# CHAINNEVERLIU/Pytorch-RL-EnhancedStableBaselines

Hardware: AMD Instinct MI355X
Metric: env-steps/sec (SAC, two-series CSTR, 4096 vec-envs) at 1/2/4/8 GPUs (higher is better)
Workload: dtype f32; 1 GPU; SAC MlpPolicy class defaults on 4096 vectorised two-series CSTR envs per GPU (obs 4/act 2, euler, batch 256, ring 244x4096, 1 gradient step per vec-step; hipGraph replay, 8 iterations per graph); n_envs_per_gpu=4096, global_batch=256, parallelism=dp1, hip_graph=True, hip_graph_requested=True, graph_unroll=8, blas=rocblas, n_updates=2370

## Files before the change

### pytorch-rl-enhancedstablebaselines_amd/csrc/cstr_chain.hip

```cpp
#include <hip/hip_runtime.h>
#include <stdint.h>

#include "../../include/cstr_rl_hip.h"
#include "cstr_device.h"
#include "cstr_rng_device.h"

namespace {

using f32x4 = __attribute__((ext_vector_type(4))) float;
typedef unsigned int u32x4 __attribute__((ext_vector_type(4)));
constexpr int BUF_OOB = 0x40000000;
constexpr int CH_THREADS = 256, CH_WAVES = 4;
constexpr float LOG_STD_MIN = -20.0f, LOG_STD_MAX = 2.0f;
constexpr int MAX_A = CSTR_MAX_HEAD_ACT;

constexpr int SM_PART = 0;
constexpr int SM_RED = SM_PART + 3 * 64 * 4;
constexpr int SM_XS = SM_RED + 4 * 16 * 8;
constexpr int SM_GS = SM_XS + 16 * 16;
constexpr int SM_PANEL = SM_GS + 16 * 8;
static size_t chain_lds_bytes(int k, int w1_pad) { return (size_t)(SM_PANEL + 16 * (k + 4) + w1_pad * k) * sizeof(float); }

__device__ __forceinline__ __amdgpu_buffer_rsrc_t rsrc_of(const float *base, const int64_t floats)
{
    return __builtin_amdgcn_make_buffer_rsrc(const_cast<float *>(base), 0, (int)(floats * 4), 0x00020000);
}

__device__ __forceinline__ float4 ld128(const __amdgpu_buffer_rsrc_t rs, const int byte_off)
{
    const u32x4 v = __builtin_amdgcn_raw_buffer_load_b128(rs, byte_off, 0, 0);
    return make_float4(__uint_as_float(v.x), __uint_as_float(v.y), __uint_as_float(v.z), __uint_as_float(v.w));
}

__device__ __forceinline__ float ld32(const __amdgpu_buffer_rsrc_t rs, const int byte_off)
{
    return __uint_as_float(__builtin_amdgcn_raw_buffer_load_b32(rs, byte_off, 0, 0));
}

template <int WX> __device__ __forceinline__ constexpr int exact_h1() { return WX == 1 ? 256 : 400; }
template <int WX> __device__ __forceinline__ constexpr int exact_h2() { return WX == 1 ? 256 : 300; }
template <int NQ, int WX> __device__ __forceinline__ constexpr int exact_tiles() { return WX == 1 ? NQ / 4 : (NQ >= 8 ? NQ / 8 : 1); }

#ifdef CSTR_CHAIN_STAMPS
__device__ unsigned long long chain_stamps[4 * 1024 * 4 * 8];
#define CH_STAMP(K, I) do { const unsigned wg_ = (blockIdx.z * gridDim.y + blockIdx.y) * gridDim.x + blockIdx.x; \
        if ((threadIdx.x & 63) == 0 && wg_ < 1024) chain_stamps[(((K) * 1024 + wg_) * 4 + (threadIdx.x >> 6)) * 8 + (I)] = __builtin_amdgcn_s_memtime(); } while (0)
#else
#define CH_STAMP(K, I) do { } while (0)
#endif

__device__ __forceinline__ void lds_barrier()
{
    __builtin_amdgcn_fence(__ATOMIC_RELEASE, "workgroup", "local");
    __builtin_amdgcn_s_barrier();
    __builtin_amdgcn_fence(__ATOMIC_ACQUIRE, "workgroup", "local");
}

__device__ __forceinline__ float rowsum16(float v)
{
    v += __int_as_float(__builtin_amdgcn_update_dpp(0, __float_as_int(v), 0x128, 0xf, 0xf, false));
    v += __int_as_float(__builtin_amdgcn_update_dpp(0, __float_as_int(v), 0x124, 0xf, 0xf, false));
    v += __int_as_float(__builtin_amdgcn_update_dpp(0, __float_as_int(v), 0x122, 0xf, 0xf, false));
    v += __int_as_float(__builtin_amdgcn_update_dpp(0, __float_as_int(v), 0x121, 0xf, 0xf, false));
    return v;
}

template <int NQ>
__device__ __forceinline__ void load_b_fwd(float4 (&bq)[NQ], const float *w, const int N, const int K, const int n0, const int ks, const int S)
{
    const int lane = threadIdx.x & 63, r = lane & 15, h = lane >> 4;
    const __amdgpu_buffer_rsrc_t rw = rsrc_of(w, (int64_t)N * K);
    const int wo = 4 * (n0 + r) * K;
#pragma unroll
    for (int u = 0; u < NQ; ++u) {
        const int k = 16 * (ks + S * u) + 4 * h;
        bq[u] = ld128(rw, (k < K && n0 + r < N) ? wo + 4 * k : BUF_OOB);
    }
}

template <int NQ>
__device__ __forceinline__ void load_b_bwd(float4 (&bq)[NQ], const float *w, const int N, const int K, const int k0, const int ks, const int S)
{
    const int lane = threadIdx.x & 63, r = lane & 15, h = lane >> 4;
    const __amdgpu_buffer_rsrc_t rw = rsrc_of(w, (int64_t)N * K);
    const bool col_ok = k0 + r < K;
#pragma unroll
    for (int u = 0; u < NQ; ++u) {
        const int n = 16 * (ks + S * u) + 4 * h;
        const int wo = 4 * (n * K + k0 + r);
        bq[u].x = ld32(rw, (col_ok && n < N) ? wo : BUF_OOB);
        bq[u].y = ld32(rw, (col_ok && n + 1 < N) ? wo + 4 * K : BUF_OOB);
        bq[u].z = ld32(rw, (col_ok && n + 2 < N) ? wo + 8 * K : BUF_OOB);
        bq[u].w = ld32(rw, (col_ok && n + 3 < N) ? wo + 12 * K : BUF_OOB);
    }
}

template <int NQ>
__device__ __forceinline__ f32x4 tile_mma(const float *panel, const int ld, const int kdim, const float4 (&bq)[NQ], const int ks, const int S)
{
    const int lane = threadIdx.x & 63, r = lane & 15, h = lane >> 4;
    f32x4 acc0 = {0.0f, 0.0f, 0.0f, 0.0f}, acc1 = acc0, acc2 = acc0, acc3 = acc0;
    float4 av[NQ];
#pragma unroll
    for (int u = 0; u < NQ; ++u) {
        const int k = 16 * (ks + S * u) + 4 * h;
        av[u] = make_float4(0.0f, 0.0f, 0.0f, 0.0f);
        if (k < kdim) av[u] = *reinterpret_cast<const float4 *>(panel + r * ld + k);
    }
#pragma unroll
    for (int u = 0; u < NQ; ++u) {
        if (16 * (ks + S * u) < kdim) {
            acc0 = __builtin_amdgcn_mfma_f32_16x16x4f32(av[u].x, bq[u].x, acc0, 0, 0, 0);
            acc1 = __builtin_amdgcn_mfma_f32_16x16x4f32(av[u].y, bq[u].y, acc1, 0, 0, 0);
            acc2 = __builtin_amdgcn_mfma_f32_16x16x4f32(av[u].z, bq[u].z, acc2, 0, 0, 0);
            acc3 = __builtin_amdgcn_mfma_f32_16x16x4f32(av[u].w, bq[u].w, acc3, 0, 0, 0);
        }
    }
    return (acc0 + acc1) + (acc2 + acc3);
}

__device__ __forceinline__ f32x4 combine_split_k(f32x4 acc, float *smem, const int T, const int S)
{
    const int lane = threadIdx.x & 63, wave = threadIdx.x >> 6;
    f32x4 *part = reinterpret_cast<f32x4 *>(smem + SM_PART);
    if (S > 1) {
        if (wave >= T) part[(wave - T) * 64 + lane] = acc;
        lds_barrier();
        if (wave < T) {
            for (int v = 1; v < S; ++v) acc += part[(wave + T * v - T) * 64 + lane];
        }
    }
    return acc;
}

constexpr int MAX_PARTS = 16;
template <int NP>
__device__ __forceinline__ float sum_parts_n(const __amdgpu_buffer_rsrc_t rs, const int n, const int64_t stride, const int64_t at)
{
    float v[NP];
#pragma unroll
    for (int p = 0; p < NP; ++p) v[p] = ld32(rs, p < n ? (int)(4 * (p * stride + at)) : BUF_OOB);
    float s = v[0];
#pragma unroll
    for (int p = 1; p < NP; ++p) s += v[p];
    return s;
}

struct PartBatch {
    float v[8];
    const float *part; int n; int64_t stride, at, total;
    __device__ __forceinline__ void request(const float *part_, const int n_, const int64_t stride_, const int64_t at_, const int64_t total_)
    {
        part = part_; n = n_; stride = stride_; at = at_; total = total_;
        const __amdgpu_buffer_rsrc_t rs = rsrc_of(part, total);
#pragma unroll
        for (int p = 0; p < 8; ++p) v[p] = ld32(rs, (p < n && n <= 8) ? (int)(4 * (p * stride + at)) : BUF_OOB);
    }
    __device__ __forceinline__ float sum() const;
};

__device__ __forceinline__ float sum_parts(const float *part, const int n, const int64_t stride, const int64_t at, const int64_t total_floats)
{
    const __amdgpu_buffer_rsrc_t rs = rsrc_of(part, total_floats);
    if (n <= 4) return sum_parts_n<4>(rs, n, stride, at);
    if (n <= 8) return sum_parts_n<8>(rs, n, stride, at);
    if (n <= MAX_PARTS) return sum_parts_n<MAX_PARTS>(rs, n, stride, at);
    float s = part[at];
    for (int p = 1; p < n; ++p) s += part[p * stride + at];
    return s;
}

__device__ __forceinline__ float PartBatch::sum() const
{
    if (n > 8) return sum_parts(part, n, stride, at, total);
    float s = v[0];
#pragma unroll
    for (int p = 1; p < 8; ++p) s += v[p];
    return s;
}

__device__ __forceinline__ void sample_action(const float mu, const float raw, const float e, float &a, float &lp_term)
{
    const float half_log_2pi = 0.91893853320467274178f;
    const float ls = fminf(fmaxf(raw, LOG_STD_MIN), LOG_STD_MAX);
    const float sd = expf(ls);
    const float u = mu + sd * e;
    a = tanhf(u);
    const float d = u - mu, var = sd * sd;
    lp_term = (-(d * d) / (2.0f * var) - logf(sd) - half_log_2pi) - logf(1.0f - a * a + 1e-6f);
}

template <int KIN>
constexpr int l1_pad() { return (KIN % 2 == 0 && KIN + 1 <= 16) ? 0 : (KIN + 1 <= 8 ? 8 : 16); }
template <int KIN>
constexpr bool l1_bias_in_k() { return KIN % 4 != 0; }

template <int KIN>
__device__ __forceinline__ float4 l1_direct_quad(const float *w1, const float *b1, const int n, const int h, float &bias)
{
    if (KIN % 4 == 0) {
        bias = b1[n];
        return 4 * h < KIN ? *reinterpret_cast<const float4 *>(w1 + (int64_t)n * KIN + 4 * h) : make_float4(0.0f, 0.0f, 0.0f, 0.0f);
    }
    bias = 0.0f;
    const int k0 = 4 * h;
    float2 lo = make_float2(0.0f, 0.0f), hi = lo;
    if (k0 + 1 < KIN) lo = *reinterpret_cast<const float2 *>(w1 + (int64_t)n * KIN + k0);
    else if (k0 == KIN) lo = make_float2(b1[n], 0.0f);
    if (k0 + 3 < KIN) hi = *reinterpret_cast<const float2 *>(w1 + (int64_t)n * KIN + k0 + 2);
    else if (k0 + 2 == KIN) hi = make_float2(b1[n], 0.0f);
    return make_float4(lo.x, lo.y, hi.x, hi.y);
}

template <int KIN>
__device__ __forceinline__ void stage_w1(float *w1s, const float *w1, const float *b1, const int h1)
{
    constexpr int KP = l1_pad<KIN>();
    if (KP == 0) return;
    for (int c = threadIdx.x; c < h1; c += CH_THREADS) {
        float w[KP > 0 ? KP : 4];
#pragma unroll
        for (int k = 0; k < KP; ++k) w[k] = k < KIN ? w1[(int64_t)c * KIN + k] : 0.0f;
        w[KP > 0 ? KIN : 0] = b1[c];
#pragma unroll
        for (int q = 0; q < KP / 4; ++q) *reinterpret_cast<float4 *>(w1s + c * KP + 4 * q) = make_float4(w[4 * q], w[4 * q + 1], w[4 * q + 2], w[4 * q + 3]);
    }
}

template <int KIN>
struct L1Direct {
    float4 wb[4];
    float bias[4];
    __device__ __forceinline__ void request(const float *w1, const float *b1, const int h1)
    {
        const int lane = threadIdx.x & 63, wave = threadIdx.x >> 6, r = lane & 15, h = lane >> 4;
#pragma unroll
        for (int i = 0; i < 4; ++i) wb[i] = l1_direct_quad<KIN>(w1, b1, min(16 * (wave + CH_WAVES * i) + r, h1 - 1), h, bias[i]);
    }
    __device__ __forceinline__ void request_flat(const float *w1, const float *b1, const int h1)
    {
        static_assert(KIN % 4 == 0, "whole-quad rows only");
        const int lane = threadIdx.x & 63, wave = threadIdx.x >> 6, r = lane & 15, h = lane >> 4;
        const __amdgpu_buffer_rsrc_t rw = rsrc_of(w1, (int64_t)h1 * KIN);
#pragma unroll
        for (int i = 0; i < 4; ++i) {
            const int n = min(16 * (wave + CH_WAVES * i) + r, h1 - 1);
            bias[i] = b1[n];
            wb[i] = ld128(rw, 4 * h < KIN ? 4 * (n * KIN + 4 * h) : BUF_OOB);
        }
    }
};

template <int KP, int KIN>
__device__ __forceinline__ void layer1_mfma(const float *xs, const float *w1s, float *panel, const int ld, const int h1,
                                            const L1Direct<KIN> *dir = nullptr, const float *w1 = nullptr, const float *b1 = nullptr)
{
    const int lane = threadIdx.x & 63, wave = threadIdx.x >> 6, r = lane & 15, h = lane >> 4;
    const bool hk = KP == 0 ? 4 * h < KIN + (l1_bias_in_k<KIN>() ? 1 : 0) : 4 * h < KP;
    const float4 zero4 = make_float4(0.0f, 0.0f, 0.0f, 0.0f);
    const float4 xa = hk ? *reinterpret_cast<const float4 *>(xs + r * 16 + 4 * h) : zero4;
    const int n_tiles = (h1 + 15) / 16;
    for (int t0 = wave; t0 < n_tiles; t0 += 4 * CH_WAVES) {
        float4 wb[4];
        float bb[4] = {0.0f, 0.0f, 0.0f, 0.0f};
#pragma unroll
        for (int i = 0; i < 4; ++i) {
            if (KP == 0) {
                if (t0 == wave) { wb[i] = dir->wb[i]; bb[i] = dir->bias[i]; }
                else wb[i] = l1_direct_quad<KIN>(w1, b1, min(16 * (t0 + CH_WAVES * i) + r, h1 - 1), h, bb[i]);
            } else {
                wb[i] = hk ? *reinterpret_cast<const float4 *>(w1s + min(16 * (t0 + CH_WAVES * i) + r, h1 - 1) * KP + 4 * h) : zero4;
            }
        }
        f32x4 acc0[4], acc1[4];
#pragma unroll
        for (int i = 0; i < 4; ++i) {
            acc0[i] = {0.0f, 0.0f, 0.0f, 0.0f};
            acc1[i] = acc0[i];
            acc0[i] = __builtin_amdgcn_mfma_f32_16x16x4f32(xa.x, wb[i].x, acc0[i], 0, 0, 0);
            acc1[i] = __builtin_amdgcn_mfma_f32_16x16x4f32(xa.y, wb[i].y, acc1[i], 0, 0, 0);
        }
#pragma unroll
        for (int i = 0; i < 4; ++i) {
            acc0[i] = __builtin_amdgcn_mfma_f32_16x16x4f32(xa.z, wb[i].z, acc0[i], 0, 0, 0);
            acc1[i] = __builtin_amdgcn_mfma_f32_16x16x4f32(xa.w, wb[i].w, acc1[i], 0, 0, 0);
        }
#pragma unroll
        for (int i = 0; i < 4; ++i) {
            const int tl = t0 + CH_WAVES * i;
            const f32x4 acc = acc0[i] + acc1[i];
            if (tl < n_tiles && 16 * tl + r < h1) {
#pragma unroll
                for (int e = 0; e < 4; ++e) panel[(4 * h + e) * ld + 16 * tl + r] = fmaxf(acc[e] + bb[i], 0.0f);
            }
        }
    }
}

__device__ __forceinline__ void store_panel(const float *panel, const int ld, float *out, const int width, const int m0)
{
    const int qpr = width / 4;
    for (int i = threadIdx.x; i < 16 * qpr; i += CH_THREADS) {
        const int row = i / qpr, q = i % qpr;
        *reinterpret_cast<float4 *>(out + (int64_t)(m0 + row) * width + 4 * q) = *reinterpret_cast<const float4 *>(panel + row * ld + 4 * q);
    }
}

struct ActorFwdArgs {
    cstr_sac_actor_t net;
    cstr_ring_t ring; int64_t *ring_ctl; int advance_ring;
    const int32_t *idx; int batch, tiles;
    float *x_data, *x_pi, *x_next, *out_done, *out_rew, *a_h1, *a_h2, *head_part;
    const uint64_t *head_rng_ctl; uint64_t head_rng_offset; float *eps_all;
    int rows_mode, head_n;
};

template <int D, int A, int NQ, int WX>
__global__ __launch_bounds__(CH_THREADS) void sac_actor_chain_fwd_kernel(const ActorFwdArgs a)
{
    extern __shared__ __align__(16) float smem[];
    constexpr int W = D + A, QPR = D / 4;
    const int t = threadIdx.x, lane = t & 63, wave = t >> 6, r = lane & 15, h = lane >> 4;
    const int T = WX ? exact_tiles<NQ, WX>() : a.tiles, S = CH_WAVES / T, tile = wave % T, ks = wave / T;
    const int H1 = WX ? exact_h1<WX>() : a.net.h1, H2 = WX ? exact_h2<WX>() : a.net.h2, B = a.batch, mode = a.rows_mode, HN = a.head_n;
    const int M = mode == CSTR_CHAIN_ROWS_PAIR ? 2 * B : B;
    const int n0 = (blockIdx.x * T + tile) * 16, m0 = blockIdx.y * 16;
    float *xs = smem + SM_XS, *red = smem + SM_RED, *panel = smem + SM_PANEL;
    const int ld = H1 + 4;
    float *w1s = panel + 16 * ld;
    const bool col_ok = n0 + r < H2;
    CH_STAMP(0, 0);
    float4 bq[NQ];
    load_b_fwd<NQ>(bq, a.net.w2, H2, H1, n0, ks, S);
    const int col = min(n0 + r, H2 - 1);
    const float bv = a.net.b2[col];
    float hwv[2 * A];
#pragma unroll
    for (int j = 0; j < 2 * A; ++j) hwv[j] = j < HN ? a.net.hw[(int64_t)j * H2 + col] : 0.0f;
    stage_w1<D>(w1s, a.net.w1, a.net.b1, H1);
    L1Direct<D> l1d;
    if (l1_pad<D>() == 0) l1d.request(a.net.w1, a.net.b1, H1);
    const bool mat = a.idx != nullptr && blockIdx.x == 0;
    float4 v = make_float4(0.0f, 0.0f, 0.0f, 0.0f), vo = v;
    float actv[A], dn = 0.0f, to = 0.0f, rw = 0.0f;
#pragma unroll
    for (int j = 0; j < A; ++j) actv[j] = 0.0f;
    int b = 0;
    bool next = false;
    const bool data_row = mode != CSTR_CHAIN_ROWS_PAIR;
    if (t < 16 * QPR) {
        const int row = t / QPR, qd = t % QPR, m = m0 + row;
        next = mode == CSTR_CHAIN_ROWS_PAIR ? m >= B : mode == CSTR_CHAIN_ROWS_NEXT;
        b = (mode == CSTR_CHAIN_ROWS_PAIR && next) ? m - B : m;
        if (a.idx) {
            const int64_t o = (int64_t)a.idx[b] * a.ring.n_envs + a.idx[B + b];
            v = *reinterpret_cast<const float4 *>((next ? a.ring.next_obs : a.ring.obs) + o * D + 4 * qd);
            if (mat && data_row && next) vo = *reinterpret_cast<const float4 *>(a.ring.obs + o * D + 4 * qd);
            if (mat && (!next || data_row) && qd == 0) {
#pragma unroll
                for (int j = 0; j < A; ++j) actv[j] = a.ring.act[o * A + j];
                dn = a.ring.done[o]; to = a.ring.timeout[o]; rw = a.ring.rew[o];
            }
        } else {
            const float2 *src = reinterpret_cast<const float2 *>((next ? a.x_next : a.x_pi) + (int64_t)b * W + 4 * qd);
            const float2 lo = src[0], hi = src[1];
            v = make_float4(lo.x, lo.y, hi.x, hi.y);
        }
        *reinterpret_cast<float4 *>(xs + row * 16 + 4 * qd) = v;
    } else if (t >= 64 && t < 64 + 16 * (4 - QPR)) {
        const int i = t - 64, row = i / (4 - QPR), qd = QPR + i % (4 - QPR);
        *reinterpret_cast<float4 *>(xs + row * 16 + 4 * qd) = make_float4(qd == QPR ? 1.0f : 0.0f, 0.0f, 0.0f, 0.0f);
    }
    constexpr int PAIRS = (A + 1) / 2;
    float e0 = 0.0f, e1 = 0.0f;
    const bool noise = a.eps_all != nullptr && blockIdx.x == 0 && wave == 3 && lane < 16 * PAIRS;
    if (noise) {
        const int row = lane / PAIRS, pr = lane % PAIRS;
        const uint64_t seed = a.head_rng_ctl[0], ctr = a.head_rng_ctl[1] + a.head_rng_offset + (uint64_t)(m0 + row);
        uint32_t rr[4];
        philox4x32_10((uint32_t)ctr, (uint32_t)(ctr >> 32), (uint32_t)pr, 0u, (uint32_t)seed, (uint32_t)(seed >> 32), rr);
        box_muller(rr[0], rr[1], e0, e1);
    }
    CH_STAMP(0, 1);
    lds_barrier();
    CH_STAMP(0, 2);
    layer1_mfma<l1_pad<D>(), D>(xs, w1s, panel, ld, H1, &l1d, a.net.w1, a.net.b1);
    lds_barrier();
    CH_STAMP(0, 3);
    f32x4 acc = tile_mma<NQ>(panel, ld, H1, bq, ks, S);
    CH_STAMP(0, 4);
    acc = combine_split_k(acc, smem, T, S);
    CH_STAMP(0, 5);
    float hv[4] = {0.0f, 0.0f, 0.0f, 0.0f};
    if (wave < T) {
#pragma unroll
        for (int e = 0; e < 4; ++e) hv[e] = col_ok ? fmaxf(acc[e] + bv, 0.0f) : 0.0f;
#pragma unroll
        for (int j = 0; j < 2 * A; ++j) {
            if (j < HN) {
#pragma unroll
                for (int e = 0; e < 4; ++e) {
// ... 320 lines not shown
    float w1a[A];
#pragma unroll
    for (int j = 0; j < A; ++j) w1a[j] = a.gact_part ? net.w1[(int64_t)col * W + D + j] : 0.0f;
    float y[2][16], w3c[2];
#pragma unroll
    for (int i = 0; i < 2; ++i) {
        const int c = min(t + CH_THREADS * i, H2 - 1);
        w3c[i] = 0.0f;
#pragma unroll
        for (int row = 0; row < 16; ++row) y[i][row] = 0.0f;
        if (i == 0 || H2 > CH_THREADS) {
            w3c[i] = net.w3[c];
#pragma unroll
            for (int row = 0; row < 16; ++row) y[i][row] = net.h2[(int64_t)(m0 + row) * H2 + c];
        }
    }
    float o_q = 0.0f, o_gq = 0.0f, o_tq = 0.0f;
    if (t < 16) {
        const bool with_alpha = rt.mode == 1 && rt.alpha.log_alpha != nullptr;
        const float ec = with_alpha ? expf(rt.alpha.log_alpha[0]) : (rt.ent_coef ? rt.ent_coef[0] : 0.0f);
        const float kq = rt.scale * 2.0f / (float)B, inv = 1.0f / (float)B;
        if (rt.mode == 1) {
            const float qa = pq[2].sum() + r_b3[2], qb = pq[3].sum() + r_b3[3];
            o_q = (g == 0 ? pq[0].sum() + r_b3[0] : pq[1].sum() + r_b3[1]);
            float q = fminf(qa, qb);
            if (rt.next_logp) q = q - ec * r_nl;
            o_tq = r_rw + (1.0f - r_dn) * rt.gamma * q;
            o_gq = kq * (o_q - o_tq);
        } else if (rt.mode == 3) {
            o_q = pq[0].sum() + r_b3[0];
            o_gq = -inv;
        } else {
            const float q1 = pq[0].sum() + r_b3[0], q2 = pq[1].sum() + r_b3[1];
            const bool first = q1 <= q2;
            o_q = g == 0 ? q1 : q2;
            o_gq = (first == (g == 0)) ? -inv : 0.0f;
        }
        gs[t] = o_gq;
    }
    CH_STAMP(2, 1);
    lds_barrier();
    CH_STAMP(2, 2);
    {
        float gq[16];
#pragma unroll
        for (int q = 0; q < 4; ++q) {
            const float4 g4 = *reinterpret_cast<const float4 *>(gs + 4 * q);
            gq[4 * q] = g4.x; gq[4 * q + 1] = g4.y; gq[4 * q + 2] = g4.z; gq[4 * q + 3] = g4.w;
        }
#pragma unroll
        for (int i = 0; i < 2; ++i) {
            const int c = t + CH_THREADS * i;
            if (c < H2) {
#pragma unroll
                for (int row = 0; row < 16; ++row) {
                    y[i][row] = y[i][row] > 0.0f ? gq[row] * w3c[i] : 0.0f;
                    panel[row * ld + c] = y[i][row];
                }
            }
        }
    }
    lds_barrier();
    CH_STAMP(2, 3);
    f32x4 acc = tile_mma<NQ>(panel, ld, H2, bq, ks, S);
    CH_STAMP(2, 4);
    acc = combine_split_k(acc, smem, T, S);
    CH_STAMP(2, 5);
    float d[4] = {0.0f, 0.0f, 0.0f, 0.0f};
    if (wave < T) {
#pragma unroll
        for (int e = 0; e < 4; ++e) d[e] = (col_ok && ty[e] > 0.0f) ? acc[e] : 0.0f;
        if (a.gact_part) {
#pragma unroll
            for (int j = 0; j < A; ++j) {
#pragma unroll
                for (int e = 0; e < 4; ++e) {
                    const float s = rowsum16(d[e] * w1a[j]);
                    if (r == 0) red[(tile * 16 + 4 * h + e) * 8 + j] = s;
                }
            }
        }
    }
    if (a.gact_part) {
        lds_barrier();
        if (t < 16 * A) {
            const int row = t / A, j = t % A;
            float s = red[row * 8 + j];
            for (int tl = 1; tl < T; ++tl) s += red[(tl * 16 + row) * 8 + j];
            a.gact_part[(((int64_t)g * gridDim.x + blockIdx.x) * B + m0 + row) * A + j] = s;
        }
    }
    CH_STAMP(2, 6);
    if (a.dz1 && wave < T && col_ok) {
#pragma unroll
        for (int e = 0; e < 4; ++e) a.dz1[((int64_t)g * B + m0 + 4 * h + e) * H1 + k0 + r] = d[e];
    }
    if (a.dz2) {
        const int cpg = (H2 + gridDim.x - 1) / gridDim.x;
#pragma unroll
        for (int i = 0; i < 2; ++i) {
            const int c = t + CH_THREADS * i;
            if (c < H2 && c / cpg == (int)blockIdx.x) {
#pragma unroll
                for (int row = 0; row < 16; ++row) a.dz2[((int64_t)g * B + m0 + row) * H2 + c] = y[i][row];
            }
        }
    }
    if (t < 16 && blockIdx.x == 0) {
        const int row = m0 + t;
        if (rt.q_out) rt.q_out[(int64_t)g * B + row] = o_q;
        if (rt.gq_out) rt.gq_out[(int64_t)g * B + row] = o_gq;
        if (rt.mode == 1 && g == 0 && rt.target_out) rt.target_out[row] = o_tq;
    }
    CH_STAMP(2, 7);
}

template <int NP>
struct PartBatchN {
    float v[NP];
    __device__ __forceinline__ void request(const float *part, const int n, const int64_t stride, const int64_t at, const int64_t total, const bool on = true)
    {
        const __amdgpu_buffer_rsrc_t rs = rsrc_of(part, total);
        const unsigned st = (unsigned)stride, at0 = (unsigned)at;
#pragma unroll
        for (int p = 0; p < NP; ++p) v[p] = ld32(rs, (on && p < n) ? (int)(4u * (p * st + at0)) : BUF_OOB);
    }
    __device__ __forceinline__ float sum() const
    {
        float s = v[0];
#pragma unroll
        for (int p = 1; p < NP; ++p) s += v[p];
        return s;
    }
};
__device__ __forceinline__ float ld_uniform(const float *p) { return ld32(rsrc_of(p, 1), 0); }

constexpr int part_bucket_row(const int n) { return n <= 8 ? 8 : 16; }
constexpr int part_bucket_loss(const int n) { return n <= 4 ? 4 : n <= 8 ? 8 : 16; }

enum { QF_PLAIN = 0, QF_GAUSSIAN = 1, QF_DETERMINISTIC = 2 };
struct QFwdLeanArgs {
    cstr_chain_net_t nets[CSTR_CHAIN_MAX_NETS];
    float *x_pi, *x_next, *params, *logp_pi, *logp_next;
};

template <int D, int A, int NQ, int FIN, int PB>
__global__ __launch_bounds__(CH_THREADS) void q_chain_fwd_lean_kernel(const int batch, const int fin_parts, const float *fin_head_part, const float *fin_hb,
                                                                      const float *fin_eps, const int fin_part_rows, const int fin_next_offset,
                                                                      const float fin_sigma, const float fin_clip, const unsigned long long roles,
                                                                      const QFwdLeanArgs a)
{
    extern __shared__ __align__(16) float smem[];
    constexpr int W = D + A, WX = 1;
    const int t = threadIdx.x, lane = t & 63, wave = t >> 6, r = lane & 15, h = lane >> 4;
    constexpr int T = exact_tiles<NQ, WX>(), S = CH_WAVES / T;
    const int tile = wave % T, ks = wave / T;
    const cstr_chain_net_t net = a.nets[blockIdx.z];
    float *const o_x_pi = a.x_pi, *const o_x_next = a.x_next, *const o_params = a.params, *const o_logp_pi = a.logp_pi, *const o_logp_next = a.logp_next;
    __builtin_amdgcn_sched_barrier(0);
    constexpr int H1 = exact_h1<WX>(), H2 = exact_h2<WX>();
    const int B = batch;
    const int n0 = (blockIdx.x * T + tile) * 16, m0 = blockIdx.y * 16;
    float *xs = smem + SM_XS, *red = smem + SM_RED, *panel = smem + SM_PANEL;
    constexpr int ld = H1 + 4;
    float *w1s = panel + 16 * ld;
    const bool col_ok = n0 + r < H2;
    CH_STAMP(1, 0);
    const int role = FIN != QF_PLAIN ? (int)((roles >> (4 * blockIdx.z)) & 15u) : CSTR_CHAIN_ROLE_PLAIN;
    const bool nxt = role == CSTR_CHAIN_ROLE_NEXT || role == CSTR_CHAIN_ROLE_NEXT_STORE;
    const bool own = nxt || role == CSTR_CHAIN_ROLE_PI;
    const bool fin_rows = own || (role == CSTR_CHAIN_ROLE_STORE_PI && blockIdx.x == 0);
    const bool fin_lane = FIN != QF_PLAIN && fin_rows && t < 16 * A;
    const int f_row = t / A, f_j = t % A;
    constexpr bool f_det = FIN == QF_DETERMINISTIC;
    PartBatchN<PB> p_mu, p_raw;
    float f_ev = 0.0f, f_hb_mu = 0.0f, f_hb_raw = 0.0f;
    constexpr int HN = f_det ? A : 2 * A;
    const int64_t f_i = (nxt ? fin_next_offset : 0) + m0 + f_row;
    if (FIN != QF_PLAIN) {
        const int64_t pstride = (int64_t)fin_part_rows * HN, ptotal = pstride * fin_parts;
        p_mu.request(fin_head_part, fin_parts, pstride, f_i * HN + f_j, ptotal, fin_lane);
        if (!f_det) p_raw.request(fin_head_part, fin_parts, pstride, f_i * HN + A + f_j, ptotal, fin_lane);
    }
    asm volatile("" ::"s"(net.w1), "s"(net.b1), "s"(net.w2), "s"(net.b2), "s"(net.w3), "s"(net.x), "s"(net.h1), "s"(net.h2), "s"(net.q_part));
    if (FIN != QF_PLAIN) asm volatile("" ::"s"(o_x_pi), "s"(o_x_next), "s"(o_params), "s"(o_logp_pi), "s"(o_logp_next));
    if (fin_lane) {
        f_ev = (!f_det || fin_eps) ? fin_eps[f_i * A + f_j] : 0.0f;
        f_hb_mu = fin_hb[f_j];
        f_hb_raw = f_det ? 0.0f : fin_hb[A + f_j];
    }
    float4 bq[NQ];
    load_b_fwd<NQ>(bq, net.w2, H2, H1, n0, ks, S);
    const int col = min(n0 + r, H2 - 1);
    const float bv = net.b2[col];
    const float w3v = col_ok ? net.w3[col] : 0.0f;
    stage_w1<W>(w1s, net.w1, net.b1, H1);
    L1Direct<W> l1d;
    if (l1_pad<W>() == 0) l1d.request(net.w1, net.b1, H1);
    {
        const int row = t >> 4, k = t & 15;
        float xv = k == W ? 1.0f : 0.0f;
        if (k < W && !(own && k >= D)) xv = net.x[(int64_t)(m0 + row) * W + k];
        if (!(own && k >= D && k < W)) xs[row * 16 + k] = xv;
    }
    float f_mu = 0.0f, f_raw = 0.0f, f_a = 0.0f, f_lp = 0.0f;
    if (fin_lane) {
        const float ev = f_ev;
        f_mu = p_mu.sum() + f_hb_mu;
        if (f_det) {
            f_a = tanhf(f_mu);
            if (nxt) f_a = fminf(fmaxf(f_a + fminf(fmaxf(ev * fin_sigma, -fin_clip), fin_clip), -1.0f), 1.0f);
        } else {
            f_raw = p_raw.sum() + f_hb_raw;
            float term;
            sample_action(f_mu, f_raw, ev, f_a, term);
            f_lp = term;
            if (A >= 2) f_lp += __shfl_xor(f_lp, 1, 64);
            if (A == 4) f_lp += __shfl_xor(f_lp, 2, 64);
        }
        if (own) xs[f_row * 16 + D + f_j] = f_a;
    }
    CH_STAMP(1, 1);
    lds_barrier();
    CH_STAMP(1, 2);
    layer1_mfma<l1_pad<W>(), W>(xs, w1s, panel, ld, H1, &l1d, net.w1, net.b1);
    lds_barrier();
    CH_STAMP(1, 3);
    f32x4 acc = tile_mma<NQ>(panel, ld, H1, bq, ks, S);
    CH_STAMP(1, 4);
    acc = combine_split_k(acc, smem, T, S);
    CH_STAMP(1, 5);
    float hv[4] = {0.0f, 0.0f, 0.0f, 0.0f};
    if (wave < T) {
#pragma unroll
        for (int e = 0; e < 4; ++e) {
            hv[e] = col_ok ? fmaxf(acc[e] + bv, 0.0f) : 0.0f;
#ifdef CSTR_HEAD_F64
            double sd = (double)hv[e] * (double)w3v;
            sd += __shfl_xor(sd, 8, 64); sd += __shfl_xor(sd, 4, 64); sd += __shfl_xor(sd, 2, 64); sd += __shfl_xor(sd, 1, 64);
            const float s = (float)sd;
#else
            const float s = rowsum16(hv[e] * w3v);
#endif
            if (r == 0) red[(tile * 16 + 4 * h + e) * 8] = s;
        }
    }
    lds_barrier();
    CH_STAMP(1, 6);
    if (t < 16) {
        float s = red[t * 8];
#pragma unroll
        for (int tl = 1; tl < T; ++tl) s += red[(tl * 16 + t) * 8];
        net.q_part[(int64_t)blockIdx.x * B + m0 + t] = s;
    }
    if (wave < T && col_ok && net.h2) {
#pragma unroll
        for (int e = 0; e < 4; ++e) net.h2[(int64_t)(m0 + 4 * h + e) * H2 + n0 + r] = hv[e];
    }
    if (blockIdx.x == 0 && net.h1) store_panel(panel, ld, net.h1, H1, m0);
    if (fin_lane && blockIdx.x == 0 && role != CSTR_CHAIN_ROLE_NEXT) {
        const int bb = m0 + f_row;
        (nxt ? o_x_next : o_x_pi)[(int64_t)bb * W + D + f_j] = f_a;
        if (!nxt && !f_det) {
            o_params[(int64_t)bb * 2 * A + f_j] = f_mu;
            o_params[(int64_t)bb * 2 * A + A + f_j] = f_raw;
        }
        if (f_j == 0 && !f_det) (nxt ? o_logp_next : o_logp_pi)[bb] = f_lp;
    }
    CH_STAMP(1, 7);
}

template <int LB>
__device__ __forceinline__ float q_from_parts_n(const float *part, const float *b3, const int n_parts, const int batch, const int row)
{
    const float b = b3[0];
    return sum_parts_n<LB>(rsrc_of(part, (int64_t)n_parts * batch), n_parts, batch, row) + b;
}

template <int MODE, bool ALPHA, bool NLOGP, int LB>
__device__ __forceinline__ void chain_loss_lean(const cstr_chain_root_t &rt, float *sm)
{
    const int tid = threadIdx.x, B = rt.batch, P = rt.n_parts;
    constexpr bool with_alpha = MODE == 1 && ALPHA;
    const float la = with_alpha ? rt.alpha.log_alpha[0] : 0.0f;
    const float ec = with_alpha ? expf(la) : (rt.ent_coef ? rt.ent_coef[0] : 0.0f);
    const float inv = 1.0f / (float)B;
    if (MODE == 1) {
        float a1 = 0.0f, a2 = 0.0f, aa = 0.0f;
        for (int b = tid; b < B; b += 256) {
            float q = fminf(q_from_parts_n<LB>(rt.q_part[2], rt.b3[2], P, B, b), q_from_parts_n<LB>(rt.q_part[3], rt.b3[3], P, B, b));
            if (NLOGP) q = q - ec * rt.next_logp[b];
            const float tq = rt.rew[b] + (1.0f - rt.done[b]) * rt.gamma * q;
            const float d1 = q_from_parts_n<LB>(rt.q_part[0], rt.b3[0], P, B, b) - tq, d2 = q_from_parts_n<LB>(rt.q_part[1], rt.b3[1], P, B, b) - tq;
            a1 += d1 * d1;
            a2 += d2 * d2;
            if (with_alpha) aa += rt.alpha.logp_pi[b] + rt.alpha.target_entropy;
        }
        const float s1 = block_sum_256(a1, sm), s2 = block_sum_256(a2, sm);
        const float mean = with_alpha ? block_sum_256(aa, sm) / (float)B : 0.0f;
        if (tid == 0) {
            const float loss = rt.scale * (s1 / (float)B + s2 / (float)B);
            if (rt.loss_out) rt.loss_out[0] = loss;
            if (rt.loss_sum) rt.loss_sum[0] += loss;
            if (with_alpha) {
                rt.alpha.grad_out[0] = -mean;
                rt.alpha.ent_coef_out[0] = ec;
                if (rt.alpha.loss_out) rt.alpha.loss_out[0] = -(la * mean);
                if (rt.alpha.loss_sum) rt.alpha.loss_sum[0] += -(la * mean);
                if (rt.alpha.ent_coef_sum) rt.alpha.ent_coef_sum[0] += ec;
            }
        }
    } else if (MODE == 3) {
        float acc = 0.0f;
        for (int b = tid; b < B; b += 256) acc += q_from_parts_n<LB>(rt.q_part[0], rt.b3[0], P, B, b);
        const float sum = block_sum_256(acc, sm);
        if (tid == 0) {
            const float loss = -(sum * inv);
            if (rt.loss_out) rt.loss_out[0] = loss;
            if (rt.loss_sum) rt.loss_sum[0] += loss;
        }
    } else {
        float acc = 0.0f;
        for (int b = tid; b < B; b += 256) {
            const float x = q_from_parts_n<LB>(rt.q_part[0], rt.b3[0], P, B, b), c = q_from_parts_n<LB>(rt.q_part[1], rt.b3[1], P, B, b);
            acc += ec * rt.logp[b] - (x <= c ? x : c);
        }
        const float sum = block_sum_256(acc, sm);
        if (tid == 0) {
            const float loss = sum * inv;
            if (rt.loss_out) rt.loss_out[0] = loss;
            if (rt.loss_sum) rt.loss_sum[0] += loss;
        }
    }
    if (tid == 0 && rt.rng_ctl) rt.rng_ctl[1] += rt.rng_advance;
    if (tid < 2 && rt.adam_advance[tid]) {
        int64_t *ctl = rt.adam_advance[tid];
        double *pw = reinterpret_cast<double *>(ctl + 2);
        ctl[0] += 1;
        pw[0] *= rt.adam_beta1[tid];
        pw[1] *= rt.adam_beta2[tid];
    }
}

struct QBwdLeanNet { const float *w1, *w2, *w3, *h1, *h2; };
struct QBwdLeanArgs {
    QBwdLeanNet nets[2];
    const float *b3[4];
    const float *ec_src;
    const float *rew, *done, *next_logp;
    float *dz2, *dz1, *gact_part, *q_out, *gq_out, *target_out;
    float gamma, scale;
    cstr_chain_root_t root;
};

template <int D, int A, int NQ, int MODE, bool ALPHA, bool NLOGP, int LB>
__global__ __launch_bounds__(CH_THREADS) void q_chain_bwd_lean_kernel(const int batch, const int n_parts, const float *qp0, const float *qp1, const float *qp2,
                                                                      const float *qp3, const QBwdLeanArgs a)
{
    extern __shared__ __align__(16) float smem[];
    constexpr int W = D + A, WX = 1;
    constexpr bool GACT = MODE != 1;
    constexpr int NEED = MODE == 1 ? 4 : MODE == 3 ? 1 : 2;
    constexpr int PB = part_bucket_row(LB);
    const int t = threadIdx.x, lane = t & 63, wave = t >> 6, r = lane & 15, h = lane >> 4;
    const int B = batch;
    constexpr int H1 = exact_h1<WX>(), H2 = exact_h2<WX>();
    const int g = blockIdx.z;
    if (__builtin_expect((int)blockIdx.y == B / 16, 0)) {
        if (g == 0 && blockIdx.x == 0) chain_loss_lean<MODE, ALPHA, NLOGP, LB>(a.root, smem + SM_RED);
        return;
    }
    constexpr int T = exact_tiles<NQ, WX>(), S = CH_WAVES / T;
    const int tile = wave % T, ks = wave / T;
    const QBwdLeanNet net = a.nets[g];
    const float *const b3p[4] = {a.b3[0], a.b3[1], a.b3[2], a.b3[3]};
    const float *const ec_src = a.ec_src, *const rew = a.rew, *const done = a.done, *const next_logp = a.next_logp;
    float *const o_dz2 = a.dz2, *const o_dz1 = a.dz1, *const o_gact = a.gact_part, *const o_q = a.q_out, *const o_gqp = a.gq_out, *const o_tqp = a.target_out;
    const float gamma = a.gamma, scale = a.scale;
    const int k0 = (blockIdx.x * T + tile) * 16, m0 = blockIdx.y * 16;
    const bool col_ok = k0 + r < H1;
    const int col = min(k0 + r, H1 - 1);
    float *red = smem + SM_RED, *gs = smem + SM_GS, *panel = smem + SM_PANEL;
    constexpr int ld = H2 + 4;
    CH_STAMP(2, 0);
    const float *const qp[4] = {qp0, qp1, qp2, qp3};
    PartBatchN<PB> pq[NEED];
    if (t < 16) {
#pragma unroll
        for (int q = 0; q < NEED; ++q) pq[q].request(qp[q], n_parts, B, m0 + t, (int64_t)n_parts * B);
    }
    asm volatile("" ::"s"(net.w1), "s"(net.w2), "s"(net.w3), "s"(net.h1), "s"(net.h2), "s"(b3p[0]), "s"(o_q), "s"(o_gqp), "s"(scale));
    if (NEED > 1) asm volatile("" ::"s"(b3p[1]));
    if (MODE == 1) asm volatile("" ::"s"(b3p[2]), "s"(b3p[3]), "s"(o_dz2), "s"(o_dz1), "s"(o_tqp), "s"(gamma), "s"(rew), "s"(done));
    if (MODE == 1 && NLOGP) asm volatile("" ::"s"(ec_src), "s"(next_logp));
    if (GACT) asm volatile("" ::"s"(o_gact));
    float r_nl = 0.0f, r_rw = 0.0f, r_dn = 0.0f, r_b3[4] = {0.0f, 0.0f, 0.0f, 0.0f}, r_ec = 0.0f;
    if (t < 16) {
        const int row = m0 + t;
#pragma unroll
        for (int q = 0; q < NEED; ++q) r_b3[q] = ld_uniform(b3p[q]);
        if (MODE == 1) {
            if (NLOGP) {
                r_nl = next_logp[row];
                r_ec = ld_uniform(ec_src);
            }
            r_rw = rew[row];
            r_dn = done[row];
        }
    }
    float4 bq[NQ];
    load_b_bwd<NQ>(bq, net.w2, H2, H1, k0, ks, S);
    float ty[4];
#pragma unroll
    for (int e = 0; e < 4; ++e) ty[e] = net.h1[(int64_t)(m0 + 4 * h + e) * H1 + col];
    float w1a[A];
#pragma unroll
    for (int j = 0; j < A; ++j) w1a[j] = GACT ? net.w1[(int64_t)col * W + D + j] : 0.0f;
    float y[16];
    const float w3c = net.w3[t];
#pragma unroll
    for (int row = 0; row < 16; ++row) y[row] = net.h2[(int64_t)(m0 + row) * H2 + t];
// ... 740 lines not shown
```

Measured before the change: 74.07 million env-steps/s.

## Defer policy-head finalisation to an idle wave and hoist prologue loads in Q forward

The lean Q-forward kernel's action-finalisation work (head sum, log-prob, output stores) now runs on the last wave, which is idle during the layer-2 reduction. Only the action needed for layer 1 is computed up front, and the log-prob is deferred. Prologue loads (eps, head bias, x input, W1 staging, direct W1 pairs via buffer loads) are issued earlier and branch-free with OOB buffer loads. This aims to shorten the serial prologue and overlap the tail work. In exchange the kernel has more complex role logic, higher register pressure from in-flight loads, and extra optional timestamp instrumentation.

```diff
diff --git a/pytorch-rl-enhancedstablebaselines_amd/csrc/cstr_chain.hip b/pytorch-rl-enhancedstablebaselines_amd/csrc/cstr_chain.hip
--- a/pytorch-rl-enhancedstablebaselines_amd/csrc/cstr_chain.hip
+++ b/pytorch-rl-enhancedstablebaselines_amd/csrc/cstr_chain.hip
@@ -30,6 +30,13 @@
 {
     const u32x4 v = __builtin_amdgcn_raw_buffer_load_b128(rs, byte_off, 0, 0);
     return make_float4(__uint_as_float(v.x), __uint_as_float(v.y), __uint_as_float(v.z), __uint_as_float(v.w));
+}
+
+__device__ __forceinline__ float2 ld64(const __amdgpu_buffer_rsrc_t rs, const int byte_off)
+{
+    typedef unsigned int u32x2 __attribute__((ext_vector_type(2)));
+    const u32x2 v = __builtin_amdgcn_raw_buffer_load_b64(rs, byte_off, 0, 0);
+    return make_float2(__uint_as_float(v.x), __uint_as_float(v.y));
 }
 
 __device__ __forceinline__ float ld32(const __amdgpu_buffer_rsrc_t rs, const int byte_off)
@@ -48,6 +55,13 @@
 #else
 #define CH_STAMP(K, I) do { } while (0)
 #endif
+#if defined(CSTR_CHAIN_STAMPS) && defined(CSTR_QFWD_FIN_STAMPS)
+#define CH_FIN_STAMPS true
+#define CH_STAMP_FIN(I, V) do { asm volatile("" ::"v"(V)); CH_STAMP(1, I); } while (0)
+#else
+#define CH_FIN_STAMPS false
+#define CH_STAMP_FIN(I, V) do { } while (0)
+#endif
 
 __device__ __forceinline__ void lds_barrier()
 {
@@ -179,15 +193,26 @@
     return s;
 }
 
+__device__ __forceinline__ void sample_action_act(const float mu, const float raw, const float e, float &a, float &sd, float &u)
+{
+    const float ls = fminf(fmaxf(raw, LOG_STD_MIN), LOG_STD_MAX);
+    sd = expf(ls);
+    u = mu + sd * e;
+    a = tanhf(u);
+}
+
+__device__ __forceinline__ float sample_action_logp(const float mu, const float sd, const float u, const float a)
+{
+    const float half_log_2pi = 0.91893853320467274178f;
+    const float d = u - mu, var = sd * sd;
+    return (-(d * d) / (2.0f * var) - logf(sd) - half_log_2pi) - logf(1.0f - a * a + 1e-6f);
+}
+
 __device__ __forceinline__ void sample_action(const float mu, const float raw, const float e, float &a, float &lp_term)
 {
-    const float half_log_2pi = 0.91893853320467274178f;
-    const float ls = fminf(fmaxf(raw, LOG_STD_MIN), LOG_STD_MAX);
-    const float sd = expf(ls);
-    const float u = mu + sd * e;
-    a = tanhf(u);
-    const float d = u - mu, var = sd * sd;
-    lp_term = (-(d * d) / (2.0f * var) - logf(sd) - half_log_2pi) - logf(1.0f - a * a + 1e-6f);
+    float sd, u;
+    sample_action_act(mu, raw, e, a, sd, u);
+    lp_term = sample_action_logp(mu, sd, u, a);
 }
 
 template <int KIN>
@@ -247,6 +272,21 @@
             const int n = min(16 * (wave + CH_WAVES * i) + r, h1 - 1);
             bias[i] = b1[n];
             wb[i] = ld128(rw, 4 * h < KIN ? 4 * (n * KIN + 4 * h) : BUF_OOB);
+        }
+    }
+    __device__ __forceinline__ void request_pairs(const float *w1, const float *b1, const int h1)
+    {
+        static_assert(KIN % 4 == 2, "rows of 4 j + 2 inputs only");
+        const int lane = threadIdx.x & 63, wave = threadIdx.x >> 6, r = lane & 15, h = lane >> 4;
+        const __amdgpu_buffer_rsrc_t rw = rsrc_of(w1, (int64_t)h1 * KIN), rb = rsrc_of(b1, h1);
+        const int k0 = 4 * h;
+#pragma unroll
+        for (int i = 0; i < 4; ++i) {
+            const int n = min(16 * (wave + CH_WAVES * i) + r, h1 - 1);
+            const float2 lo = ld64(rw, k0 + 1 < KIN ? 4 * (n * KIN + k0) : BUF_OOB), hi = ld64(rw, k0 + 3 < KIN ? 4 * (n * KIN + k0 + 2) : BUF_OOB);
+            const float bk = ld32(rb, k0 + 2 == KIN ? 4 * n : BUF_OOB);
+            bias[i] = 0.0f;
+            wb[i] = make_float4(lo.x, lo.y, k0 + 2 == KIN ? bk : hi.x, hi.y);
         }
     }
 };
@@ -873,6 +913,7 @@
 {
     extern __shared__ __align__(16) float smem[];
     constexpr int W = D + A, WX = 1;
+    constexpr bool FIN_STAMPS = CH_FIN_STAMPS && FIN != QF_PLAIN;
     const int t = threadIdx.x, lane = t & 63, wave = t >> 6, r = lane & 15, h = lane >> 4;
     constexpr int T = exact_tiles<NQ, WX>(), S = CH_WAVES / T;
     const int tile = wave % T, ks = wave / T;
@@ -890,9 +931,10 @@
     const int role = FIN != QF_PLAIN ? (int)((roles >> (4 * blockIdx.z)) & 15u) : CSTR_CHAIN_ROLE_PLAIN;
     const bool nxt = role == CSTR_CHAIN_ROLE_NEXT || role == CSTR_CHAIN_ROLE_NEXT_STORE;
     const bool own = nxt || role == CSTR_CHAIN_ROLE_PI;
-    const bool fin_rows = own || (role == CSTR_CHAIN_ROLE_STORE_PI && blockIdx.x == 0);
-    const bool fin_lane = FIN != QF_PLAIN && fin_rows && t < 16 * A;
-    const int f_row = t / A, f_j = t % A;
+    constexpr int FW = T < CH_WAVES ? CH_WAVES - 1 : 0;
+    const bool fin_store = FIN != QF_PLAIN && blockIdx.x == 0 && (role == CSTR_CHAIN_ROLE_STORE_PI || role == CSTR_CHAIN_ROLE_PI || role == CSTR_CHAIN_ROLE_NEXT_STORE);
+    const bool fin_lane = FIN != QF_PLAIN && (own || fin_store) && wave == FW && lane < 16 * A;
+    const int f_row = lane / A, f_j = lane % A;
     constexpr bool f_det = FIN == QF_DETERMINISTIC;
     PartBatchN<PB> p_mu, p_raw;
     float f_ev = 0.0f, f_hb_mu = 0.0f, f_hb_raw = 0.0f;
@@ -902,56 +944,73 @@
         const int64_t pstride = (int64_t)fin_part_rows * HN, ptotal = pstride * fin_parts;
         p_mu.request(fin_head_part, fin_parts, pstride, f_i * HN + f_j, ptotal, fin_lane);
         if (!f_det) p_raw.request(fin_head_part, fin_parts, pstride, f_i * HN + A + f_j, ptotal, fin_lane);
+        const __amdgpu_buffer_rsrc_t re = rsrc_of(fin_eps, (int64_t)fin_part_rows * A), rh = rsrc_of(fin_hb, HN);
+        f_ev = ld32(re, (fin_lane && (!f_det || fin_eps)) ? (int)(4u * (unsigned)(f_i * A + f_j)) : BUF_OOB);
+        f_hb_mu = ld32(rh, fin_lane ? 4 * f_j : BUF_OOB);
+        if (!f_det) f_hb_raw = ld32(rh, fin_lane ? 4 * (A + f_j) : BUF_OOB);
     }
     asm volatile("" ::"s"(net.w1), "s"(net.b1), "s"(net.w2), "s"(net.b2), "s"(net.w3), "s"(net.x), "s"(net.h1), "s"(net.h2), "s"(net.q_part));
     if (FIN != QF_PLAIN) asm volatile("" ::"s"(o_x_pi), "s"(o_x_next), "s"(o_params), "s"(o_logp_pi), "s"(o_logp_next));
-    if (fin_lane) {
-        f_ev = (!f_det || fin_eps) ? fin_eps[f_i * A + f_j] : 0.0f;
-        f_hb_mu = fin_hb[f_j];
-        f_hb_raw = f_det ? 0.0f : fin_hb[A + f_j];
-    }
+    const int x_row = t >> 4, x_k = t & 15;
+    const bool x_ld = x_k < W && !(own && x_k >= D);
+    const float x_in = ld32(rsrc_of(net.x, (int64_t)B * W), x_ld ? 4 * ((m0 + x_row) * W + x_k) : BUF_OOB);
+    stage_w1<W>(w1s, net.w1, net.b1, H1);
+    L1Direct<W> l1d;
+    if constexpr (W % 4 == 2) l1d.request_pairs(net.w1, net.b1, H1);
+    else if (l1_pad<W>() == 0) l1d.request(net.w1, net.b1, H1);
     float4 bq[NQ];
     load_b_fwd<NQ>(bq, net.w2, H2, H1, n0, ks, S);
     const int col = min(n0 + r, H2 - 1);
     const float bv = net.b2[col];
     const float w3v = col_ok ? net.w3[col] : 0.0f;
-    stage_w1<W>(w1s, net.w1, net.b1, H1);
-    L1Direct<W> l1d;
-    if (l1_pad<W>() == 0) l1d.request(net.w1, net.b1, H1);
-    {
-        const int row = t >> 4, k = t & 15;
-        float xv = k == W ? 1.0f : 0.0f;
-        if (k < W && !(own && k >= D)) xv = net.x[(int64_t)(m0 + row) * W + k];
-        if (!(own && k >= D && k < W)) xs[row * 16 + k] = xv;
-    }
-    float f_mu = 0.0f, f_raw = 0.0f, f_a = 0.0f, f_lp = 0.0f;
-    if (fin_lane) {
-        const float ev = f_ev;
+    if (!(own && x_k >= D && x_k < W)) xs[x_row * 16 + x_k] = x_ld ? x_in : (x_k == W ? 1.0f : 0.0f);
+    float f_mu = 0.0f, f_raw = 0.0f, f_a = 0.0f, f_sd = 0.0f, f_u = 0.0f;
+    const auto fin_action = [&]() {
         f_mu = p_mu.sum() + f_hb_mu;
+        CH_STAMP_FIN(3, f_mu);
         if (f_det) {
             f_a = tanhf(f_mu);
-            if (nxt) f_a = fminf(fmaxf(f_a + fminf(fmaxf(ev * fin_sigma, -fin_clip), fin_clip), -1.0f), 1.0f);
+            if (nxt) f_a = fminf(fmaxf(f_a + fminf(fmaxf(f_ev * fin_sigma, -fin_clip), fin_clip), -1.0f), 1.0f);
         } else {
             f_raw = p_raw.sum() + f_hb_raw;
-            float term;
-            sample_action(f_mu, f_raw, ev, f_a, term);
-            f_lp = term;
-            if (A >= 2) f_lp += __shfl_xor(f_lp, 1, 64);
-            if (A == 4) f_lp += __shfl_xor(f_lp, 2, 64);
-        }
-        if (own) xs[f_row * 16 + D + f_j] = f_a;
+            sample_action_act(f_mu, f_raw, f_ev, f_a, f_sd, f_u);
+        }
+    };
+    const auto fin_deferred = [&]() {
+        if (fin_lane && fin_store) {
+            if (!own) fin_action();
+            const int bb = m0 + f_row;
+            (nxt ? o_x_next : o_x_pi)[(int64_t)bb * W + D + f_j] = f_a;
+            if (!f_det) {
+                if (!nxt) {
+                    o_params[(int64_t)bb * 2 * A + f_j] = f_mu;
+                    o_params[(int64_t)bb * 2 * A + A + f_j] = f_raw;
+                }
+                float f_lp = sample_action_logp(f_mu, f_sd, f_u, f_a);
+                if (A >= 2) f_lp += __shfl_xor(f_lp, 1, 64);
+                if (A == 4) f_lp += __shfl_xor(f_lp, 2, 64);
+                CH_STAMP_FIN(5, f_lp);
+                if (f_j == 0) (nxt ? o_logp_next : o_logp_pi)[bb] = f_lp;
+            }
+        }
+    };
+    if (fin_lane && own) {
+        fin_action();
+        xs[f_row * 16 + D + f_j] = f_a;
+        CH_STAMP_FIN(4, f_a);
     }
     CH_STAMP(1, 1);
     lds_barrier();
     CH_STAMP(1, 2);
     layer1_mfma<l1_pad<W>(), W>(xs, w1s, panel, ld, H1, &l1d, net.w1, net.b1);
     lds_barrier();
-    CH_STAMP(1, 3);
+    if (!FIN_STAMPS) CH_STAMP(1, 3);
     f32x4 acc = tile_mma<NQ>(panel, ld, H1, bq, ks, S);
-    CH_STAMP(1, 4);
+    if (!FIN_STAMPS) CH_STAMP(1, 4);
     acc = combine_split_k(acc, smem, T, S);
-    CH_STAMP(1, 5);
+    if (!FIN_STAMPS) CH_STAMP(1, 5);
     float hv[4] = {0.0f, 0.0f, 0.0f, 0.0f};
+    if (FW != 0 && wave == FW) fin_deferred();
     if (wave < T) {
 #pragma unroll
         for (int e = 0; e < 4; ++e) {
@@ -979,15 +1038,7 @@
         for (int e = 0; e < 4; ++e) net.h2[(int64_t)(m0 + 4 * h + e) * H2 + n0 + r] = hv[e];
     }
     if (blockIdx.x == 0 && net.h1) store_panel(panel, ld, net.h1, H1, m0);
-    if (fin_lane && blockIdx.x == 0 && role != CSTR_CHAIN_ROLE_NEXT) {
-        const int bb = m0 + f_row;
-        (nxt ? o_x_next : o_x_pi)[(int64_t)bb * W + D + f_j] = f_a;
-        if (!nxt && !f_det) {
-            o_params[(int64_t)bb * 2 * A + f_j] = f_mu;
-            o_params[(int64_t)bb * 2 * A + A + f_j] = f_raw;
-        }
-        if (f_j == 0 && !f_det) (nxt ? o_logp_next : o_logp_pi)[bb] = f_lp;
-    }
+    if (FW == 0) fin_deferred();
     CH_STAMP(1, 7);
 }
 
```

New measurement: 77.64 million env-steps/s (median of 6 runs). +4.8%, better.
